# clearmatics/libff

Hardware: AMD Instinct MI355X
Metric: G1 MSM throughput (scalar-muls/sec) (higher is better)
Workload: dtype u32

## Files before the change

libff_amd/csrc/engine.cpp:

```cpp
#include "../../include/amdmsm.h"
#include "engine_internal.h"
#include "group_vtable.h"
#include "fr_vtable.h"

#include <hip/hip_runtime.h>

#include <fcntl.h>
#include <sys/stat.h>
#include <unistd.h>

#include <algorithm>
#include <atomic>
#include <cmath>
#include <cstdio>
#include <cstdlib>
#include <cstring>
#include <initializer_list>
#include <mutex>
#include <string>
#include <thread>
#include <utility>
#include <vector>

using namespace amdmsm;

constexpr int MAX_SLOTS = 4;
constexpr int MAX_GROUPS = 4;
struct ws_slot {
    void *ws = nullptr;
    size_t ws_bytes = 0;
    hipEvent_t done = nullptr;
    bool used = false;
    hipStream_t side[MAX_GROUPS - 1] = {};
    hipEvent_t acc_done[MAX_GROUPS - 1] = {}, tail_done[MAX_GROUPS - 1] = {};
    long long last_ticket = -1;
    bool ev_valid = false;
    hipEvent_t ov_in = nullptr, ov_acc = nullptr, ov_tail = nullptr;
};

struct grow_buf {
    void *p = nullptr;
    size_t bytes = 0;
};

struct base_entry {
    uint64_t id = 0;
    int curve = 0, group = 0, form = 0;
    const char *host = nullptr;
    size_t n = 0, stride = 0;
    void *d_aff = nullptr;
    void *d_endo = nullptr;
    bool automatic = false;
    bool pinned = false;
    uint64_t last_use = 0;
    size_t aff_bytes = 0;
    size_t bytes() const { return n * aff_bytes * (d_endo ? 2 : 1); }
};

struct fb_state {
    grow_buf small, table, table_aff, out;
    bool valid = false;
    int curve = 0, group = 0;
    size_t scalar_size = 0, window = 0;
    unsigned char g[3 * 24 * 2 * 4] = {};
};

struct stream_state {
    static constexpr int NB = 2;
    void *h_stage[NB] = {};
    size_t h_bytes[NB] = {};
// ... 284 lines not shown
    place(p.big, &off, batch, p.c <= 22 ? align_up(std::max(sort_geometry(n, p.c, p.W).big_words, big_words_min) * 4, 256) : 256);
    place(p.tmp_payload, &off, Wt, p.list_stride * 4);
    place(p.tmp_key, &off, Wt, p.list_stride * 4);
    place(p.endo, &off, batch, glv ? align_up((n / 2) * (size_t)vt->el_words * 2 * 4, 256) : 0);
    {
        static const int rc_env = getenv("AMDMSM_ROWCOL") ? atoi(getenv("AMDMSM_ROWCOL")) : 1;
        static const int rc_min_c = getenv("AMDMSM_ROWCOL_MIN_C") ? atoi(getenv("AMDMSM_ROWCOL_MIN_C")) : 10;
        static const int qr_env = getenv("AMDMSM_ROWCOL_QROW") ? atoi(getenv("AMDMSM_ROWCOL_QROW")) : 0;
        static const int qc_env = getenv("AMDMSM_ROWCOL_QCOL") ? atoi(getenv("AMDMSM_ROWCOL_QCOL")) : 0;
        p.rowcol = rc_env != 0 && p.c >= rc_min_c;
        const int h = p.c / 2;
        const size_t C = (size_t)1 << h, R = p.B >> h;
        const bool one_wave = vt->fq_words >= 24 || vt->el_words > vt->fq_words;
        const size_t lane_budget = one_wave ? 70000 : 140000;
        uint32_t q = 4;
        while (q < 64 && Wt * p.B * red_lanes * 2 / q > lane_budget) q <<= 1;
        p.q_row = qr_env > 0 ? (uint32_t)qr_env : q;
        p.q_col = qc_env > 0 ? (uint32_t)qc_env : q;
        place(p.rc, &off, Wt, (R + 1 + C) * xyz_bytes);
        place(p.planes, &off, Wt, p.c * xyz_bytes);
        place(p.winsum, &off, Wt, xyz_bytes);
    }
    p.total = off;
    return AMDMSM_OK;
}

int ensure_ws(amdmsm_ctx *ctx, ws_slot &sl, size_t bytes) {
    if (sl.ws_bytes >= bytes) return AMDMSM_OK;
    if (sl.ws) {
        HIP_TRY(ctx, hipDeviceSynchronize());
        HIP_TRY(ctx, hipFree(sl.ws));
        sl.ws = nullptr;
        sl.ws_bytes = 0;
    }
    const size_t want = bytes + bytes / 8;
    HIP_TRY(ctx, hipMalloc(&sl.ws, want));
    sl.ws_bytes = want;
    return AMDMSM_OK;
}

constexpr uint64_t TIMING_RING = 64;
hipError_t timing_event(hipEvent_t *e) {
    static const bool nofence = !(getenv("AMDMSM_TIMING_NOFENCE") && atoi(getenv("AMDMSM_TIMING_NOFENCE")) == 0);
    return nofence ? hipEventCreateWithFlags(e, hipEventDisableSystemFence) : hipEventCreate(e);
}
void record(amdmsm_ctx *ctx, ws_slot &, int idx, hipStream_t st) {
    if (ctx->timing) (void)hipEventRecord(ctx->ring[ctx->ticket % TIMING_RING][idx], st);
}

int glv_env() {
    static const int env = [] {
        const char *e = getenv("AMDMSM_GLV");
        int v = 0;
        if (!e) return 0;
        if (!strcmp(e, "off") || !strcmp(e, "0")) v = -1;
        else if (!strcmp(e, "on") || !strcmp(e, "1")) v = 1;
        else if (!strcmp(e, "all") || !strcmp(e, "force") || !strcmp(e, "2")) v = 2;
        else if (!strcmp(e, "auto")) v = 3;
        if (v) fprintf(stderr, "[amdmsm] AMDMSM_GLV=%s overrides amdmsm_opts.endomorphism where the caller left it at 0 "
                               "(off: everywhere); on / force assert that every base lies in the order-r subgroup\n", e);
        return v;
    }();
    return env;
}
int endomorphism_permitted(const group_vtable *vt, const amdmsm_opts *opts) {
    const int env = glv_env();
// ... 38 lines not shown
    return (opts && opts->stream) ? (hipStream_t)opts->stream : ctx->stream;
}
amdmsm_opts opts_or_default(const amdmsm_opts *opts) {
    amdmsm_opts o = AMDMSM_OPTS_INIT;
    if (opts) o = *opts;
    else o.out_form = AMDMSM_OUT_LIBFF;
    return o;
}

constexpr size_t MAX_RANGES = 64;
size_t max_range_points() {
    static const size_t v = [] {
        const char *e = getenv("AMDMSM_MAX_RANGE_POINTS");
        const long long x = e ? atoll(e) : 0;
        return x > 0 ? (size_t)x : (size_t)1 << 28;
    }();
    return v;
}

struct msm_hook {
    int (*fn)(void *arg, hipEvent_t *wait_for) = nullptr;
    void *arg = nullptr;
};
struct short_spec {
    int kind = 0;
    int bits = 0;
    uint32_t *flag = nullptr;
    bool uploaded = false;
    size_t elem_bytes(const group_vtable *vt) const { return kind ? (size_t)kind : (size_t)vt->fr_words * 4; }
};
int short_limit_bits(const group_vtable *vt, const short_spec &ss) {
    return ss.flag ? ss.bits : (ss.kind ? 8 * ss.kind : 32 * vt->fr_words);
}
uint32_t *enqueue_tail(const group_vtable *vt, const plan_t &p, char *ws, int w0, int nw, hipStream_t ts, int queue) {
    const size_t w = (size_t)w0;
    uint32_t *buckets = ws_at(ws, p.buckets, w);
    vt->accumulate_fixup(ts, ws_at(ws, p.counts, w), buckets, ws_at(ws, p.pfirst, w), ws_at(ws, p.plast, w), ws_at(ws, p.cont, w),
                         ws_at(ws, p.queue, (size_t)queue), nw, p.B, p.S, p.T);
    if (p.rowcol) {
        uint32_t *winsum = ws_at(ws, p.winsum, w);
        vt->reduce_rowcol(ts, buckets, nw, p.B, p.c, p.q_row, p.q_col, ws_at(ws, p.rc, w), ws_at(ws, p.planes, w), winsum);
        return winsum;
    }
    uint32_t *src = ws_at(ws, p.lvl0, w), *dst = ws_at(ws, p.lvl1, w);
    vt->reduce_segments(ts, buckets, nw, p.B, p.L, src);
    const uint32_t fold = (uint32_t)vt->reduce_fold;
    uint32_t M = p.B / p.L;
    M /= std::min<uint32_t>(M, fold);
    while (M > 1) {
        if ((size_t)M * (64 / fold) <= 256) {
            vt->sum_block(ts, src, nw, M, dst);
            M = 1;
        } else {
            vt->sum_butterfly(ts, src, nw, M, dst);
            M /= std::min<uint32_t>(M, fold);
        }
        std::swap(src, dst);
    }
    return src;
}

int msm_device_impl(amdmsm_ctx *ctx, const group_vtable *vt, const uint32_t *d_bases, const uint32_t *d_scalars,
                    size_t n, uint32_t *d_out, const amdmsm_opts *opts, int table_digits = 0,
                    const msm_hook *hook = nullptr, const uint32_t *d_endo_resident = nullptr, const short_spec *ss = nullptr) {
    hipStream_t st = stream_of(ctx, opts);
    hipStream_t const user_st = st;
    const int form = opts ? opts->out_form : AMDMSM_OUT_LIBFF;
    const int mont = (opts && opts->scalars_plain) ? 0 : 1;
    static const bool atomic_env = getenv("AMDMSM_SORT") && !strcmp(getenv("AMDMSM_SORT"), "atomic");
    const bool atomic_sort = atomic_env && !ss;
    const bool glv = !ss && use_endomorphism(vt, n, opts, table_digits) && !atomic_sort;
// ... 5 lines not shown
        return AMDMSM_OK;
    }
    plan_t p;
    static const int acc_s_env = getenv("AMDMSM_ACC_S") ? atoi(getenv("AMDMSM_ACC_S")) : 0;
    static const int groups_env = getenv("AMDMSM_WINDOW_GROUPS") ? atoi(getenv("AMDMSM_WINDOW_GROUPS")) : 0;
    static const bool overlap_env = getenv("AMDMSM_OVERLAP") && atoi(getenv("AMDMSM_OVERLAP")) != 0;
    const bool overlap = overlap_env && ctx->depth > 1 && ctx->bulk_stream && vt->accumulate_overlap_ok && !groups_env;
    plan_req req;
    req.entries = entries;
    req.c = opts ? opts->window_bits : 0;
    req.L = opts ? opts->segment_len : 0;
    req.S = acc_s_env;
    req.table_digits = table_digits;
    req.groups = groups_env;
    req.glv = glv;
    req.overlap = overlap;
    req.sbits = ss ? ss->bits : 0;
    int rc = make_plan(vt, req, p);
    if (rc) return fail(ctx, rc, "bad window_bits / segment_len");
    if (ss && p.c > 22) return fail(ctx, AMDMSM_ERR_BAD_ARG, "window_bits > 22 is not available for short scalars");
    const int slot_idx = (int)(ctx->next++ % (unsigned)ctx->depth);
    ws_slot &sl = ctx->slots[slot_idx];
    ctx->last_slot = slot_idx;
    if (overlap) {
        HIP_TRY(ctx, hipEventRecord(sl.ov_in, user_st));
        st = ctx->bulk_stream;
        HIP_TRY(ctx, hipStreamWaitEvent(st, sl.ov_in, 0));
    }
    if (sl.used) HIP_TRY(ctx, hipStreamWaitEvent(st, sl.done, 0));
    rc = ensure_ws(ctx, sl, p.total);
    if (rc) return rc;
    char *ws = (char *)sl.ws;
    const sort_bufs sb = sort_bufs_of(p, ws, 0);

    record(ctx, sl, 0, st);
    const uint32_t *endo_pts = !glv ? nullptr : (d_endo_resident ? d_endo_resident : ws_at(ws, p.endo));
    const bool endo_beside = glv && !d_endo_resident && !(hook && hook->fn);
    HIP_TRY(ctx, hipEventRecord(sl.tail_done[0], st));
    if ((atomic_sort || p.c > 22) && !table_digits) {
        HIP_TRY(ctx, hipMemsetAsync(sb.ends, 0, (size_t)p.W * p.counts.unit, st));
        vt->count(st, d_scalars, n, mont, p.c, p.W, sb.ends);
        record(ctx, sl, 1, st);
        vt->scatter(st, d_scalars, n, mont, p.c, p.W, sb.ends, sb.lists, p.list_stride);
    } else {
        HIP_TRY(ctx, hipMemsetAsync(sb.coarse, 0, p.big.off + 16 - p.coarse.off, st));
        record(ctx, sl, 1, st);
        if (ss)
            vt->sort(st, sort_src::short_scalars(d_scalars, ss->kind, short_limit_bits(vt, *ss), ss->flag), n, mont, p.c, p.W, sb, 0);
        else
            vt->sort(st, sort_src::own(d_scalars), n, mont, p.c, table_digits ? table_digits : p.W, sb,
                     table_digits ? 1 : (glv ? 2 : 0));
    }
    hipStream_t side = overlap ? st : sl.side[0];
    if (!overlap) HIP_TRY(ctx, hipStreamWaitEvent(side, sl.tail_done[0], 0));
    HIP_TRY(ctx, hipMemsetAsync(ws_at(ws, p.buckets), 0, (size_t)p.W * p.buckets.unit, side));
    for (int g = 0; g < p.G; ++g) HIP_TRY(ctx, hipMemsetAsync(ws_at(ws, p.queue, (size_t)g), 0, 8, side));
    if (endo_beside) vt->endo_points(side, d_bases, n, ws_at(ws, p.endo));
    if (!overlap) HIP_TRY(ctx, hipEventRecord(sl.acc_done[0], side));
    if (hook && hook->fn) {
        hipEvent_t wait_for = nullptr;
        rc = hook->fn(hook->arg, &wait_for);
        if (rc) return rc;
        if (wait_for) HIP_TRY(ctx, hipStreamWaitEvent(st, wait_for, 0));
    }
    if (!overlap) HIP_TRY(ctx, hipStreamWaitEvent(st, sl.acc_done[0], 0));
    if (glv && !d_endo_resident && !endo_beside) vt->endo_points(st, d_bases, n, ws_at(ws, p.endo));
    int w_hi = p.W;
    for (int g = 0; g < p.G; ++g) {
        const int wg = p.W / p.G + (g < p.W % p.G ? 1 : 0);
        const int w0 = w_hi - wg;
        w_hi = w0;
        const bool last = g == p.G - 1;
        hipStream_t ts = last ? (overlap ? ctx->tail_stream : st) : sl.side[g];
        if (g == 0) record(ctx, sl, 2, st);
        vt->accumulate(st, ws_at(ws, p.counts, w0), ws_at(ws, p.lists, w0), p.list_stride, d_bases, ws_at(ws, p.buckets, w0),
                       ws_at(ws, p.pfirst, w0), ws_at(ws, p.plast, w0), ws_at(ws, p.cont, w0), wg, p.B, p.S, p.T, endo_pts, n,
                       overlap ? 1 : 0);
        if (last) {
            record(ctx, sl, 3, st);
            if (overlap) {
                HIP_TRY(ctx, hipEventRecord(sl.ov_acc, st));
                HIP_TRY(ctx, hipStreamWaitEvent(ts, sl.ov_acc, 0));
            }
        } else {
            HIP_TRY(ctx, hipEventRecord(sl.acc_done[g], st));
            HIP_TRY(ctx, hipStreamWaitEvent(ts, sl.acc_done[g], 0));
        }
        const uint32_t *src = enqueue_tail(vt, p, ws, w0, wg, ts, g);
        if (g > 0) HIP_TRY(ctx, hipStreamWaitEvent(ts, sl.tail_done[g - 1], 0));
        if (last) record(ctx, sl, 4, ts);
        vt->horner(ts, src, wg, p.c, last ? form : (int)AMDMSM_OUT_JACOBIAN, g > 0 ? ws_at(ws, p.partial, g - 1) : nullptr,
                   last ? d_out : ws_at(ws, p.partial, g));
        if (!last) HIP_TRY(ctx, hipEventRecord(sl.tail_done[g], ts));
    }
    if (overlap) {
        record(ctx, sl, 5, ctx->tail_stream);
        HIP_TRY(ctx, hipEventRecord(sl.ov_tail, ctx->tail_stream));
        HIP_TRY(ctx, hipStreamWaitEvent(user_st, sl.ov_tail, 0));
        st = user_st;
    } else {
        record(ctx, sl, 5, st);
    }
    if (ctx->timing) sl.last_ticket = (long long)ctx->ticket++;
    sl.ev_valid = ctx->timing;
    HIP_TRY(ctx, hipEventRecord(sl.done, st));
    sl.used = true;
    HIP_TRY(ctx, hipGetLastError());
    return AMDMSM_OK;
}

constexpr int MAX_BATCH = 8;
int ensure_buf(amdmsm_ctx *ctx, grow_buf &b, size_t bytes);

struct item_dev {
    const uint32_t *bases = nullptr;
    size_t n = 0;
    const uint32_t *scalars = nullptr;
    size_t offset = 0;
    const uint32_t *index = nullptr;
    uint32_t *out = nullptr;
};

int msm_device_batch_items_impl(amdmsm_ctx *ctx, const group_vtable *vt, int k, const item_dev *it, const uint32_t *d_shared,
                                size_t shared_n, uint32_t *flags, const amdmsm_opts *opts) {
    hipStream_t st = stream_of(ctx, opts);
    const int form = opts ? opts->out_form : AMDMSM_OUT_LIBFF;
    const int mont = (opts && opts->scalars_plain) ? 0 : 1;
    size_t n_max = 0;
    for (int j = 0; j < k; ++j) n_max = std::max(n_max, it[j].n);
    if (flags) HIP_TRY(ctx, hipMemsetAsync(flags, 0, (size_t)k * 4, st));
    if (n_max == 0) {
        for (int j = 0; j < k; ++j) vt->sum_points(st, it[j].out, 0, form, it[j].out);
        HIP_TRY(ctx, hipGetLastError());
        return AMDMSM_OK;
    }
    const bool glv = use_endomorphism(vt, n_max, opts, 0);
    const size_t entries = glv ? 2 * n_max : n_max;
    plan_req req;
    req.entries = entries;
    req.c = opts ? opts->window_bits : 0;
    req.L = opts ? opts->segment_len : 0;
    req.glv = glv;
    req.batch = k;
    plan_t p;
    int rc = make_plan(vt, req, p);
    if (rc) return fail(ctx, rc, "bad window_bits / segment_len");
    if (p.c > 22) return fail(ctx, AMDMSM_ERR_BAD_ARG, "window_bits > 22 is not available for a batch");
    req.c = p.c;
    for (int j = 0; j < k; ++j) {
        if (it[j].n) req.big_words_min = std::max(req.big_words_min, sort_geometry(glv ? 2 * it[j].n : it[j].n, p.c, p.W).big_words);
    }
    rc = make_plan(vt, req, p);
    if (rc) return fail(ctx, rc, "bad window_bits / segment_len");
    const int slot_idx = (int)(ctx->next++ % (unsigned)ctx->depth);
    ws_slot &sl = ctx->slots[slot_idx];
    ctx->last_slot = slot_idx;
    if (sl.used) HIP_TRY(ctx, hipStreamWaitEvent(st, sl.done, 0));
    rc = ensure_ws(ctx, sl, p.total);
    if (rc) return rc;
    char *ws = (char *)sl.ws;
    const size_t Wt = (size_t)p.W * (size_t)k;
    record(ctx, sl, 0, st);
    HIP_TRY(ctx, hipMemsetAsync(ws_at(ws, p.coarse), 0, p.big.off - p.coarse.off, st));
    for (int j = 0; j < k; ++j) HIP_TRY(ctx, hipMemsetAsync(ws_at(ws, p.big, (size_t)j), 0, 16, st));
    HIP_TRY(ctx, hipMemsetAsync(ws_at(ws, p.buckets), 0, Wt * p.buckets.unit, st));
    HIP_TRY(ctx, hipMemsetAsync(ws_at(ws, p.queue), 0, 8, st));
    record(ctx, sl, 1, st);
    bool first = true;
    for (int j = 0; j < k; ++j) {
        const size_t w0 = (size_t)j * p.W, n = it[j].n;
        const sort_bufs sb = sort_bufs_of(p, ws, (size_t)j);
        if (n == 0) {
            HIP_TRY(ctx, hipMemsetAsync(sb.ends, 0, (size_t)p.W * p.counts.unit, st));
            HIP_TRY(ctx, hipMemsetAsync(ws_at(ws, p.cont, w0), 0xff, (size_t)p.W * p.cont.unit, st));
            continue;
        }
        const sort_src src_j = it[j].scalars ? sort_src::own(it[j].scalars)
                                             : sort_src::selected(d_shared, shared_n, it[j].index, it[j].offset, flags + j);
        vt->sort(st, src_j, n, mont, p.c, p.W, sb, glv ? 2 : 0);
        uint32_t *endo_j = glv ? ws_at(ws, p.endo, (size_t)j) : nullptr;
        if (glv) vt->endo_points(st, it[j].bases, n, endo_j);
        if (first) record(ctx, sl, 2, st);
        first = false;
        vt->accumulate(st, sb.ends, sb.lists, p.list_stride, it[j].bases, ws_at(ws, p.buckets, w0), ws_at(ws, p.pfirst, w0),
                       ws_at(ws, p.plast, w0), ws_at(ws, p.cont, w0), p.W, p.B, p.S, p.T, endo_j, n, 0);
    }
    record(ctx, sl, 3, st);
    const uint32_t *src = enqueue_tail(vt, p, ws, 0, (int)Wt, st, 0);
    record(ctx, sl, 4, st);
    uint32_t *outs[MAX_BATCH];
// ... 1929 lines not shown

struct vec_opts {
    int mont, form, kernel_form;
};
vec_opts vec_opts_of(const amdmsm_opts *opts) {
    const int form = opts ? opts->out_form : AMDMSM_OUT_LIBFF;
    return {(opts && opts->scalars_plain) ? 0 : 1, form, form == AMDMSM_OUT_AFFINE ? (int)AMDMSM_OUT_LIBFF : form};
}
void vec_finish(const group_vtable *vt, hipStream_t st, const vec_opts &vo, uint32_t *d_xyz, size_t n, uint32_t *scratch) {
    if (vo.form != AMDMSM_OUT_AFFINE) return;
    vt->import_bases(st, d_xyz, (size_t)vt->el_words * 3, 0, n, scratch);
    vt->export_affine(st, scratch, n, d_xyz);
}

int vec_check_stride(amdmsm_ctx *ctx, const group_vtable *vt, size_t &stride_bytes, const char *what) {
    const size_t xyz_bytes = (size_t)vt->el_words * 12;
    if (stride_bytes == 0) stride_bytes = xyz_bytes;
    if (stride_bytes % rec_align(vt) || stride_bytes < xyz_bytes) return fail(ctx, AMDMSM_ERR_BAD_ARG, what);
    return AMDMSM_OK;
}
int vec_upload(amdmsm_ctx *ctx, const group_vtable *vt, hipStream_t st, const void *points_xyz, size_t stride_bytes, int base_form,
               size_t first, size_t m, void *d_aff) {
    HIP_TRY(ctx, hipMemcpyAsync(ctx->hb_src.p, (const char *)points_xyz + first * stride_bytes,
                                (m - 1) * stride_bytes + (size_t)vt->el_words * 12, hipMemcpyHostToDevice, st));
    vt->import_bases(st, (const uint32_t *)ctx->hb_src.p, stride_bytes / 4, base_form == AMDMSM_FORM_SPECIAL, m, (uint32_t *)d_aff);
    return AMDMSM_OK;
}

int slot_begin(amdmsm_ctx *ctx, hipStream_t st, size_t bytes, ws_slot *&slp) {
    const int slot_idx = (int)(ctx->next++ % (unsigned)ctx->depth);
    ws_slot &sl = ctx->slots[slot_idx];
    ctx->last_slot = slot_idx;
    if (sl.used) HIP_TRY(ctx, hipStreamWaitEvent(st, sl.done, 0));
    slp = &sl;
    return ensure_ws(ctx, sl, bytes);
}
int slot_end(amdmsm_ctx *ctx, hipStream_t st, ws_slot &sl) {
    record(ctx, sl, 5, st);
    if (ctx->timing) sl.last_ticket = (long long)ctx->ticket++;
    sl.ev_valid = ctx->timing;
    HIP_TRY(ctx, hipEventRecord(sl.done, st));
    sl.used = true;
    return AMDMSM_OK;
}

template <class Chunk>
int vec_run_chunks(amdmsm_ctx *ctx, const group_vtable *vt, hipStream_t st, size_t ws_bytes, size_t n, size_t cn, void *h_out,
                   Chunk &&chunk) {
    const size_t xyz_bytes = (size_t)vt->el_words * 12;
    ws_slot *sl = nullptr;
    int rc = slot_begin(ctx, st, ws_bytes, sl);
    if (rc) return rc;
    record(ctx, *sl, 0, st);
    for (size_t off = 0; off < n; off += cn) {
        const size_t m = n - off < cn ? n - off : cn;
        rc = chunk(*sl, off, m, off == 0);
        if (rc) {
            if (h_out) (void)hipDeviceSynchronize();
            return rc;
        }
        if (h_out) HIP_TRY(ctx, hipMemcpyAsync((char *)h_out + off * xyz_bytes, ctx->fb.out.p, m * xyz_bytes, hipMemcpyDeviceToHost, st));
        if (off == 0) record(ctx, *sl, 4, st);
        if (h_out) HIP_TRY(ctx, hipStreamSynchronize(st));
    }
    return slot_end(ctx, st, *sl);
}
// ... 1941 lines not shown
```

libff_amd/csrc/group_vtable.h:

```cpp
#pragma once
#include <hip/hip_runtime_api.h>
#include <stddef.h>
#include <stdint.h>
#include <stdlib.h>

namespace amdmsm {

enum out_form : int {
    OUT_JACOBIAN = 0,
    OUT_LIBFF = 1,
    OUT_AFFINE = 2,
};

struct sort_geom {
    int hb;
    int fb;
    uint32_t chunk_cap;
    uint32_t big_thresh;
    uint32_t big_cap;
    size_t big_words;
};
constexpr int SORT_HB_MAX = 10;
constexpr size_t SORT_COARSE_WORDS = ((size_t)1 << SORT_HB_MAX) + 1, SORT_CURSOR_WORDS = (size_t)1 << SORT_HB_MAX;
inline sort_geom sort_geometry(size_t n, int c, int W) {
// ... 111 lines not shown
    const uint32_t* glv_lambda;

    void (*import_bases)(hipStream_t, const uint32_t* src, size_t stride_words, int form_special,
                         size_t n, uint32_t* dst_affine);
    void (*export_affine)(hipStream_t, const uint32_t* src_affine, size_t n, uint32_t* dst_xyz);
    void (*gen_bases_seq)(hipStream_t, unsigned long long first, size_t n, uint32_t* dst_affine);
    void (*endo_points)(hipStream_t, const uint32_t* bases_affine, size_t n, uint32_t* out);
    void (*precompute_table)(hipStream_t, const uint32_t* bases_affine, size_t n, int c, int D, uint32_t* tmp,
                             uint32_t* table);
    void (*ffi_decode_points)(hipStream_t, const uint32_t* src_be, size_t n, uint32_t* dst_affine, uint32_t* status);
    void (*ffi_decode_scalars)(hipStream_t, const uint32_t* src_be, size_t n, uint32_t* dst_plain, uint32_t* status);
    void (*ffi_encode_point)(hipStream_t, const uint32_t* src_xyz_affine, uint32_t* dst_be);
    void (*disk_decode)(hipStream_t, const uint32_t* src, size_t n, uint32_t* dst_affine);
    void (*disk_decode_compressed)(hipStream_t, const uint32_t* src, size_t n, uint32_t* dst_affine, uint32_t* status);

    void (*scalar_stats)(hipStream_t, const uint32_t* scalars, size_t n, int mont, uint32_t* stats);
    void (*scalar_bits)(hipStream_t, const void* scalars, int kind, size_t n, int mont, uint32_t* out_bits);
    void (*gather_scalars)(hipStream_t, const uint32_t* shared, size_t shared_n, const uint32_t* index, size_t offset,
                           uint32_t* flag, size_t n, uint32_t* out);
    void (*count)(hipStream_t, const uint32_t* scalars, size_t n, int mont, int c, int W, uint32_t* counts);
    void (*scatter)(hipStream_t, const uint32_t* scalars, size_t n, int mont, int c, int W, uint32_t* cursor,
                    uint32_t* lists, size_t list_stride);
    void (*sort)(hipStream_t, const sort_src& src, size_t n, int mont, int c, int W, const sort_bufs& bufs, int mode);
    int (*sort_top_window)(int mode, int mont, int c, int W, size_t columns, int* tb);

    void (*accumulate)(hipStream_t, const uint32_t* ends, const uint32_t* lists, size_t list_stride,
                       const uint32_t* bases_affine, uint32_t* buckets, uint32_t* part_first, uint32_t* part_last,
                       uint32_t* cont_bucket, int W, uint32_t B, uint32_t S, uint32_t T, const uint32_t* endo_points,
                       size_t n_real, int overlap);
    size_t (*accumulate_resident_lanes)(int overlap);
    int accumulate_overlap_ok;
    void (*accumulate_fixup)(hipStream_t, const uint32_t* ends, uint32_t* buckets, uint32_t* part_first,
                             const uint32_t* part_last, const uint32_t* cont_bucket, uint32_t* queue, int W,
                             uint32_t B, uint32_t S, uint32_t T);

    void (*reduce_segments)(hipStream_t, const uint32_t* buckets, int W, uint32_t B, uint32_t L, uint32_t* out);
    void (*sum_butterfly)(hipStream_t, const uint32_t* in, int W, uint32_t M, uint32_t* out);
    void (*sum_block)(hipStream_t, const uint32_t* in, int W, uint32_t M, uint32_t* out);
    void (*reduce_rowcol)(hipStream_t, const uint32_t* buckets, int W, uint32_t B, int c, uint32_t q_row, uint32_t q_col,
                          uint32_t* rc, uint32_t* planes, uint32_t* out);
    void (*horner)(hipStream_t, const uint32_t* window_sums, int W, int c, int form, const uint32_t* init,
                   uint32_t* out);
    void (*horner_batch)(hipStream_t, const uint32_t* window_sums, int k, int W, int c, int form, uint32_t* const* outs);
    void (*sum_points)(hipStream_t, const uint32_t* pts, int k, int form, uint32_t* out);

    void (*fixed_base_exp)(hipStream_t, const uint32_t* g_xyz, int scalar_size, int window, const uint32_t* scalars,
                           size_t n, int mont, const uint32_t* coeff, int form, uint32_t* gouter, uint32_t* table,
                           uint32_t* table_aff, int build_table, uint32_t* out);

    int smv_entries;
    void (*smv_table)(hipStream_t, const uint32_t* bases_affine, size_t n, uint32_t* tmp, uint32_t* table);
    void (*smv_ladder)(hipStream_t, const uint32_t* table, size_t n, const uint32_t* scalars, int mont, int form, uint32_t* out);

    int seg_windows, seg_digit_stride;
    void (*seg_digits)(hipStream_t, const uint32_t* scalars, size_t n, int mont, uint32_t* digits);
    void (*seg_accumulate)(hipStream_t, const uint32_t* table, size_t nt, const uint32_t* digits, const uint32_t* slices,
                           size_t n_slices, uint32_t* sums);
    void (*seg_fold)(hipStream_t, const uint32_t* sums, const uint32_t* seg_first, size_t m, uint32_t* winsum);
    void (*seg_horner)(hipStream_t, const uint32_t* winsum, size_t m, int form, uint32_t* out);

    int fold_digit_stride;
    void (*fold_digits)(hipStream_t, const uint32_t* scalars_host, int k, int mont, int glv, int W, uint32_t* digits);
    void (*fold_ladder)(hipStream_t, const uint32_t* tables, size_t n, const uint32_t* digits, int rows, int glv, int W,
                        int form, uint32_t* out);

    void (*fft_gather)(hipStream_t, const uint32_t* in_affine, size_t b0, size_t cn, int rsh, uint32_t* dst_affine);
    void (*fft_butterfly)(hipStream_t, const uint32_t* table, size_t cn, const uint32_t* in_affine, size_t b0, int rsh,
// ... 43 lines not shown
```

libff_amd/csrc/msm_group.hip:

```cpp
#include "curve_params.h"
#include "ec.cuh"
#include "fp2h.cuh"
#include "group_vtable.h"
#include "wide.cuh"
#include "wide28.cuh"
#include "rr.cuh"

#include <algorithm>
#include <cstdio>
#include <vector>
#include <type_traits>

#ifndef AMDMSM_GROUP
#error "compile with -DAMDMSM_GROUP=<group traits> -DAMDMSM_VT=<vtable getter name>"
#endif

namespace amdmsm {
template <bool I>
struct ec_coeff_a<Fp<AMDMSM_GROUP::fq, I>> {
    static constexpr int value = AMDMSM_GROUP::DEG == 1 ? AMDMSM_GROUP::COEFF_A : 0;
};
template <int NR, bool I>
struct ec_coeff_a<Fp2<AMDMSM_GROUP::fq, NR, I>> {
    static constexpr int value = AMDMSM_GROUP::DEG == 2 ? AMDMSM_GROUP::COEFF_A : 0;
// ... 868 lines not shown
    __shared__ uint32_t tmp[NT / 64 + 1];
    const uint32_t nbin = 1u << hb;
    const uint32_t bin = blockIdx.x, w = blockIdx.y;
    const bool top = dtop != 0 && w == gridDim.y - 1u;
    const int fb = c - 1 - hb - (top ? dtop : 0);
    const uint32_t nfine = 1u << fb, fmask = nfine - 1u;
    uint32_t* fstart = smem;
    uint32_t* chist = fstart + nfine;
    uint32_t* cstart = chist + nfine;
    uint32_t* ccur = cstart + nfine;
    uint32_t* st_payload = ccur + nfine;
    unsigned short* st_fine = reinterpret_cast<unsigned short*>(st_payload + chunk_cap);
    const uint32_t* cs = coarse + (size_t)w * (nbin + 1);
    const uint32_t b0 = __builtin_amdgcn_readfirstlane(cs[bin]), m = __builtin_amdgcn_readfirstlane(cs[bin + 1]) - b0;
    const sort_key_t* key = tmp_key + (size_t)w * stride + b0;
    const uint32_t* pay = tmp_payload + (size_t)w * stride + b0;
    uint32_t* out = lists + (size_t)w * stride + b0;
    uint32_t* e = ends + (((size_t)w << (c - 1)) + ((size_t)bin << fb));
    if (top) {
        const uint32_t share = (1u << (fb + dtop)) - nfine, total = cs[nbin];
        uint32_t* tail = ends + (((size_t)w << (c - 1)) + ((size_t)nbin << fb) + (size_t)bin * share);
        for (uint32_t j = threadIdx.x; j < share; j += NT) tail[j] = total;
    }
    if (m > big_thresh) {
        for (uint32_t j = threadIdx.x; j < nfine; j += NT) e[j] = 0;
        if (threadIdx.x == 0) {
            const uint32_t tiles = (m + SORT_TILE - 1) / SORT_TILE;
            const uint32_t slot = atomicAdd(&big[0], 1u);
            uint32_t* rec = big + 4 + 4 * (size_t)slot;
            rec[0] = w;
            rec[1] = bin;
            rec[2] = atomicAdd(&big[1], tiles);
            rec[3] = tiles;
        }
        return;
    }
    if (m <= chunk_cap) {
        uint32_t fr[PER];
        if (m == 0) {
            for (uint32_t j = threadIdx.x; j < nfine; j += NT) e[j] = b0;
            return;
        }
        for (uint32_t j = threadIdx.x; j < nfine; j += NT) chist[j] = 0;
#pragma unroll
        for (int q = 0; q < PER; ++q) {
            const uint32_t k = threadIdx.x + (uint32_t)q * NT;
            fr[q] = (uint32_t)key[k < m ? k : m - 1u] & fmask;
        }
        __syncthreads();
#pragma unroll
        for (int q = 0; q < PER; ++q) {
            const uint32_t k = threadIdx.x + (uint32_t)q * NT;
            const uint32_t r = k < m ? atomicAdd(&chist[fr[q]], 1u) : 0u;
            fr[q] = r | (fr[q] << 14);
        }
        __syncthreads();
        block_exclusive_scan<NT, (1 << SORT_MAX_FB) / NT>(chist, fstart, nfine, tmp);
        for (uint32_t j = threadIdx.x; j < nfine; j += NT) e[j] = b0 + fstart[j] + chist[j];
#pragma unroll
        for (int q = 0; q < PER; ++q) {
            const uint32_t k = threadIdx.x + (uint32_t)q * NT;
            if (k < m) st_payload[fstart[fr[q] >> 14] + (fr[q] & 0x3fffu)] = pay[k];
        }
        __syncthreads();
        for (uint32_t k = threadIdx.x; k < m; k += NT) out[k] = st_payload[k];
        return;
// ... 49 lines not shown
        }
        __syncthreads();
        for (uint32_t j = threadIdx.x; j < nfine; j += NT) fstart[j] += hist_c[j];
        __syncthreads();
    }
}

struct big_tile {
    uint32_t rec, w, bin, k0, cm;
};
AMDMSM_DEV bool big_find_tile(const uint32_t* __restrict__ big, const uint32_t* __restrict__ coarse, uint32_t nbin,
                              uint32_t tile, uint32_t* sh, big_tile& bt, uint32_t& b0) {
    const uint32_t nbig = big[0];
    __syncthreads();
    for (uint32_t r = threadIdx.x; r < nbig; r += SORT_TPB) {
        const uint32_t* rec = big + 4 + 4 * (size_t)r;
        if (tile >= rec[2] && tile < rec[2] + rec[3]) sh[0] = r;
    }
    __syncthreads();
    bt.rec = sh[0];
    const uint32_t* rec = big + 4 + 4 * (size_t)bt.rec;
    bt.w = rec[0];
    bt.bin = rec[1];
    const uint32_t* cs = coarse + (size_t)bt.w * (nbin + 1);
    b0 = cs[bt.bin];
    const uint32_t m = cs[bt.bin + 1] - b0;
    bt.k0 = (tile - rec[2]) * SORT_TILE;
    bt.cm = (m - bt.k0 < (uint32_t)SORT_TILE) ? m - bt.k0 : (uint32_t)SORT_TILE;
    return true;
}

__global__ void __launch_bounds__(SORT_TPB) k_sort_big_hist(const sort_key_t* __restrict__ tmp_key,
                                                            const uint32_t* __restrict__ coarse, size_t stride, int c,
                                                            int hb, const uint32_t* __restrict__ big,
                                                            uint32_t* __restrict__ ends, uint32_t wtop, int dtop) {
    __shared__ uint32_t hist[1 << SORT_MAX_FB], sh[1];
    const uint32_t nbin = 1u << hb;
    const uint32_t tiles = big[1];
    for (uint32_t tile = blockIdx.x; tile < tiles; tile += gridDim.x) {
        big_tile bt;
        uint32_t b0;
        big_find_tile(big, coarse, nbin, tile, sh, bt, b0);
        const int fb = c - 1 - hb - (bt.w == wtop ? dtop : 0);
        const uint32_t nfine = 1u << fb, fmask = nfine - 1u;
        for (uint32_t j = threadIdx.x; j < nfine; j += SORT_TPB) hist[j] = 0;
        __syncthreads();
        const sort_key_t* key = tmp_key + (size_t)bt.w * stride + b0 + bt.k0;
        for (uint32_t k = threadIdx.x; k < bt.cm; k += SORT_TPB) atomicAdd(&hist[key[k] & fmask], 1u);
        __syncthreads();
        uint32_t* e = ends + (((size_t)bt.w << (c - 1)) + ((size_t)bt.bin << fb));
        for (uint32_t j = threadIdx.x; j < nfine; j += SORT_TPB)
            if (hist[j]) atomicAdd(&e[j], hist[j]);
    }
}

__global__ void __launch_bounds__(SORT_TPB) k_sort_big_scan(const uint32_t* __restrict__ coarse, int c, int hb,
                                                            uint32_t big_cap, uint32_t* __restrict__ big,
                                                            uint32_t* __restrict__ ends, uint32_t wtop, int dtop) {
    __shared__ uint32_t cnt[1 << SORT_MAX_FB], out[1 << SORT_MAX_FB], tmp[SORT_TPB / 64 + 1];
    const uint32_t nbin = 1u << hb;
    const int fb_row = c - 1 - hb;
    const uint32_t nbig = big[0];
    for (uint32_t r = blockIdx.x; r < nbig; r += gridDim.x) {
        const uint32_t* rec = big + 4 + 4 * (size_t)r;
        const uint32_t w = rec[0], bin = rec[1];
        const uint32_t b0 = coarse[(size_t)w * (nbin + 1) + bin];
        const int fb = fb_row - (w == wtop ? dtop : 0);
        const uint32_t nfine = 1u << fb;
        uint32_t* e = ends + (((size_t)w << (c - 1)) + ((size_t)bin << fb));
        uint32_t* cur = big + 4 + 4 * (size_t)big_cap + ((size_t)r << fb_row);
        __syncthreads();
        for (uint32_t j = threadIdx.x; j < nfine; j += SORT_TPB) cnt[j] = e[j];
        __syncthreads();
        block_exclusive_scan(cnt, out, nfine, tmp);
        for (uint32_t j = threadIdx.x; j < nfine; j += SORT_TPB) {
            cur[j] = b0 + out[j];
            e[j] = b0 + out[j] + cnt[j];
        }
    }
}

__global__ void __launch_bounds__(SORT_TPB, SORT_WAVES_2WG) k_sort_big_scatter(const uint32_t* __restrict__ tmp_payload,
                                                               const sort_key_t* __restrict__ tmp_key,
                                                               const uint32_t* __restrict__ coarse, size_t stride, int c,
                                                               int hb, uint32_t big_cap, uint32_t* __restrict__ big,
// ... 420 lines not shown
        acc_add(acc, pi >= n_real ? endo_pts + (size_t)(pi - n_real) * AFFW : bases + (size_t)pi * AFFW, (ent >> 31) != 0);
    }
#endif
    if (bend == hi) {
        acc_store(from_prev ? part_first + g * ZZS : bk + (size_t)b * ZZS, acc);
        cont_bucket[g] = NO_BUCKET;
    } else if (from_prev) {
        acc_store(part_first + g * ZZS, acc);
        cont_bucket[g] = NO_BUCKET;
    } else {
        acc_store(part_last + g * ZZS, acc);
        cont_bucket[g] = b;
    }
}

AMDMSM_DEV void wave_group_sum(Jac<E>& p, uint32_t G);
AMDMSM_DEV void wave_group_sum_r(Jac<ER>& p, uint32_t G);

#ifdef AMDMSM_INLINE_SPAN
constexpr uint32_t INLINE_SPAN = AMDMSM_INLINE_SPAN;
#else
constexpr uint32_t INLINE_SPAN = FQ::N <= 8 ? 3 : 2;
#endif
constexpr uint32_t MID_SPAN = 32;
constexpr uint32_t MID_G = 8;

AMDMSM_DEV uint32_t* fixup_queue_base(uint32_t* q, size_t lanes, int mid) {
    return q + 2 + (mid ? 2 * fixup_queue_cap_long(lanes) : 0);
}

AMDMSM_DEV void fixup_compact_block(uint32_t blk, const uint32_t* __restrict__ ends, uint32_t* __restrict__ part_first, int W,
                                    uint32_t B, uint32_t S, uint32_t T);

__global__ void __launch_bounds__(64, AMDMSM_TAIL_WAVES) k_accumulate_fixup(const uint32_t* __restrict__ ends,
                                                         uint32_t* __restrict__ part_first,
                                                         const uint32_t* __restrict__ part_last,
                                                         const uint32_t* __restrict__ cont_bucket,
                                                         uint32_t* __restrict__ buckets, uint32_t* __restrict__ queue,
                                                         int W, uint32_t B, uint32_t S, uint32_t T, uint32_t fix_blocks) {
    if (blockIdx.x >= fix_blocks) {
        fixup_compact_block(blockIdx.x - fix_blocks, ends, part_first, W, B, S, T);
        return;
    }
    const size_t g = gtid() / RED_LANES;
    const bool first_of_pair = (threadIdx.x % RED_LANES) == 0;
    const size_t w = g / T;
    const uint32_t t = (uint32_t)(g % T);
    uint32_t b = NO_BUCKET, t_last = 0;
    if (w < (size_t)W) {
        b = cont_bucket[g];
        if (b != NO_BUCKET) t_last = (ends[w * B + b] - 1) / S;
    }
    const uint32_t span = (b != NO_BUCKET) ? t_last - t : 0;
    const size_t lanes = (size_t)W * T;
#pragma unroll
    for (int mid = 0; mid < 2; ++mid) {
        const bool mine = first_of_pair && (mid ? (span > INLINE_SPAN && span <= MID_SPAN) : (span > MID_SPAN));
        const unsigned long long m = __ballot(mine);
        if (m == 0) continue;
        const uint32_t lane = threadIdx.x & 63u;
        uint32_t base = 0;
        if (lane == (uint32_t)__ffsll((long long)m) - 1u) base = atomicAdd(&queue[mid], (uint32_t)__popcll(m));
        base = (uint32_t)__shfl((int)base, __ffsll((long long)m) - 1, 64);
        if (mine) {
            const uint32_t slot = base + (uint32_t)__popcll(m & ((1ull << lane) - 1ull));
            uint32_t* q = fixup_queue_base(queue, lanes, mid);
            q[2 * (size_t)slot] = (uint32_t)g;
            q[2 * (size_t)slot + 1] = (uint32_t)(g >> 32);
        }
    }
    if (span == 0 || span > INLINE_SPAN) return;
    rec_sum sum;
// ... 1872 lines not shown
    if (split_hist && sg.chunk_cap >= 16384 && ((size_t)16 << sg.fb) * 4 <= 32768) perchunk_words = 16u << sg.fb;
    const size_t fine_lds = ((size_t)4 << sg.fb) * 4 + (size_t)sg.chunk_cap * 6 + (size_t)perchunk_words * 4;
    const size_t big_lds = ((size_t)4 << sg.fb) * 4 + (size_t)SORT_TILE * 4;
    static const bool reported = [&] {
        if (!(getenv("AMDMSM_SORT_REPORT") && atoi(getenv("AMDMSM_SORT_REPORT")))) return false;
        int k16 = 0, k32 = 0, kf = 0, kb = 0;
        (void)hipOccupancyMaxActiveBlocksPerMultiprocessor(&k16, k_sort_coarse<unsigned short>, SORT_TPB, 0);
        (void)hipOccupancyMaxActiveBlocksPerMultiprocessor(&k32, k_sort_coarse<uint32_t>, SORT_TPB, 0);
        if (sg.chunk_cap <= 8192)
            (void)hipOccupancyMaxActiveBlocksPerMultiprocessor(&kf, k_sort_fine<SORT_TPB, 8>, SORT_TPB, fine_lds);
        else if (sg.chunk_cap <= 12288)
            (void)hipOccupancyMaxActiveBlocksPerMultiprocessor(&kf, k_sort_fine<SORT_TPB, 12>, SORT_TPB, fine_lds);
        else
            (void)hipOccupancyMaxActiveBlocksPerMultiprocessor(&kf, k_sort_fine<SORT_TPB, 16>, SORT_TPB, fine_lds);
        (void)hipOccupancyMaxActiveBlocksPerMultiprocessor(&kb, k_sort_big_scatter, SORT_TPB, big_lds);
        fprintf(stderr, "[amdmsm sort] workgroups per CU: k_sort_coarse 16-bit keys %d, 32-bit keys %d; k_sort_fine<1024> "
                        "(chunk_cap %u, %zu B of LDS) %d; k_sort_big_scatter (%zu B) %d\n",
                k16, k32, sg.chunk_cap, fine_lds, kf, big_lds, kb);
        return true;
    }();
    (void)reported;
#define AMDMSM_LAUNCH_FINE(NT, PER)                                                                                          \
    hipLaunchKernelGGL((k_sort_fine<NT, PER>), dim3(nbin, We), dim3(NT), fine_lds, st, b.tmp_payload, tmp_key16, b.coarse, b.stride, c, \
                       hb, sg.chunk_cap, sg.big_thresh, sg.big_cap, perchunk_words, b.big, b.ends, b.lists, dtop)
    if (sg.chunk_cap <= 4096)
        AMDMSM_LAUNCH_FINE(256, 16);
    else if (sg.chunk_cap <= 8192)
        AMDMSM_LAUNCH_FINE(SORT_TPB, 8);
    else if (sg.chunk_cap <= 12288)
        AMDMSM_LAUNCH_FINE(SORT_TPB, 12);
    else
        AMDMSM_LAUNCH_FINE(SORT_TPB, 16);
#undef AMDMSM_LAUNCH_FINE
    hipLaunchKernelGGL(k_sort_big_hist, dim3(512), dim3(SORT_TPB), 0, st, tmp_key16, b.coarse, b.stride, c, hb, b.big, b.ends, wtop, dtop);
    hipLaunchKernelGGL(k_sort_big_scan, dim3(256), dim3(SORT_TPB), 0, st, b.coarse, c, hb, sg.big_cap, b.big, b.ends, wtop, dtop);
    hipLaunchKernelGGL(k_sort_big_scatter, dim3(512), dim3(SORT_TPB), big_lds, st, b.tmp_payload, tmp_key16, b.coarse, b.stride, c,
                       hb, sg.big_cap, b.big, b.lists, wtop, dtop);
}
void l_scalar_bits(hipStream_t st, const void* scalars, int kind, size_t n, int mont, uint32_t* out) {
    if (!n) return;
    const size_t items = kind == 1 ? packed_items<1>(scalars, n) : kind == 2 ? packed_items<2>(scalars, n)
                         : kind == 4 ? packed_items<4>(scalars, n) : kind == 8 ? packed_items<8>(scalars, n) : n;
    const dim3 grid((unsigned)std::min<size_t>((items + TPB - 1) / TPB, 4096));
    if (kind == 1) hipLaunchKernelGGL(k_scalar_bits<1>, grid, dim3(TPB), 0, st, scalars, n, mont, out);
    else if (kind == 2) hipLaunchKernelGGL(k_scalar_bits<2>, grid, dim3(TPB), 0, st, scalars, n, mont, out);
    else if (kind == 4) hipLaunchKernelGGL(k_scalar_bits<4>, grid, dim3(TPB), 0, st, scalars, n, mont, out);
    else if (kind == 8) hipLaunchKernelGGL(k_scalar_bits<8>, grid, dim3(TPB), 0, st, scalars, n, mont, out);
    else hipLaunchKernelGGL(k_scalar_bits<0>, grid, dim3(TPB), 0, st, scalars, n, mont, out);
}
void l_gather_scalars(hipStream_t st, const uint32_t* shared, size_t shared_n, const uint32_t* index, size_t offset,
                      uint32_t* flag, size_t n, uint32_t* out) {
    if (!n) return;
    hipLaunchKernelGGL(k_gather_scalars, dim3(blocks_for(n)), dim3(TPB), 0, st, shared, n, index, offset, shared_n, flag, out);
}
size_t l_accumulate_resident_lanes(int overlap);
constexpr size_t ACC_OVERLAP_LDS = AMDMSM_ACC_WAVES >= 3 ? (160 * 1024) / AMDMSM_ACC_WAVES - 16 * 1024 + 1024 : 0;
void l_accumulate(hipStream_t st, const uint32_t* ends, const uint32_t* lists, size_t list_stride, const uint32_t* bases,
                  uint32_t* buckets, uint32_t* part_first, uint32_t* part_last, uint32_t* cont_bucket, int W, uint32_t B,
                  uint32_t S, uint32_t T, const uint32_t* endo_pts, size_t n_real, int overlap) {
    overlap = overlap && AMDMSM_OVERLAP_OK && ACC_OVERLAP_LDS;
    int sync_waves = (size_t)W * T * ACC_LANES <= 2 * l_accumulate_resident_lanes(overlap) * ACC_LANES ? 1 : 0;
    if (overlap) sync_waves = 2;
    const size_t dyn_lds = overlap ? ACC_OVERLAP_LDS : 0;
#ifdef AMDMSM_ACC_TRACE
    {
        const size_t waves = (size_t)blocks_for((size_t)W * T * ACC_LANES) * TPB / 64;
        static unsigned long long* d_trace = nullptr;
        static size_t cap = 0;
// ... 13 lines not shown
            if (FILE* f = fopen(path, "wb")) {
                fwrite(h.data(), 8, h.size(), f);
                fclose(f);
            }
        }
    }
#else
    hipLaunchKernelGGL(k_accumulate, dim3(blocks_for((size_t)W * T * ACC_LANES)), dim3(TPB), dyn_lds, st, ends, lists,
                       list_stride, bases, buckets, part_first, part_last, cont_bucket, W, B, S, T, endo_pts,
                       endo_pts ? (uint32_t)n_real : 0x80000000u, sync_waves);
#endif
}
void l_endo_points(hipStream_t st, const uint32_t* bases, size_t n, uint32_t* out) {
    if (!n) return;
    hipLaunchKernelGGL(k_endo_points, dim3(blocks_for(n * 2 * GP::DEG)), dim3(TPB), 0, st, bases, n, out);
}
void l_glv_digits(hipStream_t st, const uint32_t* scalars, size_t n, int mont, int c, int W, int32_t* out) {
    if (!n) return;
    hipLaunchKernelGGL(k_glv_digits, dim3(blocks_for(n)), dim3(TPB), 0, st, scalars, n, mont, c, W, out);
}
size_t l_accumulate_resident_lanes(int overlap) {
    auto query = [](size_t dyn_lds) {
        int dev = 0, cus = 256, blocks = 0;
        if (hipGetDevice(&dev) == hipSuccess) (void)hipDeviceGetAttribute(&cus, hipDeviceAttributeMultiprocessorCount, dev);
        if (hipOccupancyMaxActiveBlocksPerMultiprocessor(&blocks, k_accumulate, TPB, dyn_lds) != hipSuccess || blocks <= 0) blocks = 4;
        return (size_t)cus * (size_t)blocks * TPB / ACC_LANES;
    };
    static const size_t lanes = query(0);
    static const size_t lanes_overlap = (AMDMSM_OVERLAP_OK && ACC_OVERLAP_LDS) ? query(ACC_OVERLAP_LDS) : lanes;
    return overlap ? lanes_overlap : lanes;
}
void l_accumulate_fixup(hipStream_t st, const uint32_t* ends, uint32_t* buckets, uint32_t* part_first,
                        const uint32_t* part_last, const uint32_t* cont_bucket, uint32_t* queue, int W, uint32_t B,
                        uint32_t S, uint32_t T) {
    const unsigned fix_blocks = blocks_for((size_t)W * T * RED_LANES, 64);
    const unsigned compact_blocks = T / FIX_BLOCK >= 2 ? (unsigned)(W * (T / FIX_BLOCK - 1)) : 0u;
    hipLaunchKernelGGL(k_accumulate_fixup, dim3(fix_blocks + compact_blocks), dim3(64), 0, st, ends, part_first,
                       part_last, cont_bucket, buckets, queue, W, B, S, T, fix_blocks);
    const size_t lanes = (size_t)W * T;
    const size_t cap_mid = fixup_queue_cap_mid(lanes) / (RED_FOLD / MID_G) + 1, cap_long = fixup_queue_cap_long(lanes);
    const unsigned mid_blocks = (unsigned)(cap_mid < 8192 ? cap_mid : 8192), long_blocks = (unsigned)(cap_long < 2048 ? cap_long : 2048);
    hipLaunchKernelGGL(k_accumulate_fixup_queue, dim3(mid_blocks + long_blocks), dim3(64), 0, st, ends,
                       part_first, part_last, cont_bucket, buckets, queue, mid_blocks, lanes, B, S, T);
}
void l_reduce_segments(hipStream_t st, const uint32_t* buckets, int W, uint32_t B, uint32_t L, uint32_t* out) {
    hipLaunchKernelGGL(k_reduce_segments, dim3(blocks_for((size_t)W * (B / L) * RED_LANES, 64)), dim3(64), 0, st, buckets, W, B,
                       L, out);
}
void l_sum_butterfly(hipStream_t st, const uint32_t* in, int W, uint32_t M, uint32_t* out) {
    hipLaunchKernelGGL(k_sum_butterfly, dim3(blocks_for((size_t)W * M * RED_LANES, 64)), dim3(64), 0, st, in, W, M, out);
}
void l_sum_block(hipStream_t st, const uint32_t* in, int W, uint32_t M, uint32_t* out) {
    if (M >= 8 && M * RED_LANES <= (uint32_t)SUMW_THREADS && (M & (M - 1)) == 0) {
        hipLaunchKernelGGL(k_sum_block_wide, dim3(W), dim3(SUMW_THREADS), 0, st, in, W, M, out);
        return;
    }
    const unsigned threads = (unsigned)((M * RED_LANES + 63) / 64 * 64);
    hipLaunchKernelGGL(k_sum_block, dim3(W), dim3(threads), 0, st, in, W, M, out);
}
void l_reduce_rowcol(hipStream_t st, const uint32_t* buckets, int W, uint32_t B, int c, uint32_t q_row, uint32_t q_col,
                     uint32_t* rc, uint32_t* planes, uint32_t* out) {
    const int h = c / 2;
    const uint32_t C = 1u << h, R = B >> h;
    auto fit = [](uint32_t len, uint32_t q) {
        if (q < 1) q = 1;
        while (q & (q - 1)) q &= q - 1;
        if (q > len) q = len;
        while (len / q > RED_FOLD) q <<= 1;
        return q;
    };
    q_row = fit(C, q_row);
// ... 224 lines not shown
```

Baseline: 664.7 million.

## Fold sort-buffer clearing into fixup kernel and merge big-bin scan into histogram

Instead of a separate memset of the sort scratch region at the start of each MSM, the fixup kernel of the previous call on the same slot gets extra blocks that zero that region, and the next call skips the memset when the slot is known clean. The big-bin histogram kernel also performs the per-record exclusive scan in whichever block finishes last for that record, using an atomic arrival counter, so the separate k_sort_big_scan launch is dropped. This removes a memset and a kernel launch from the critical path. In exchange it relies on cross-call slot state, threadfence-based last-block detection and extra counter storage in the big buffer, which raises correctness risk.

```diff
diff --git a/libff_amd/csrc/engine.cpp b/libff_amd/csrc/engine.cpp
--- a/libff_amd/csrc/engine.cpp
+++ b/libff_amd/csrc/engine.cpp
@@ -36,6 +36,8 @@
     long long last_ticket = -1;
     bool ev_valid = false;
     hipEvent_t ov_in = nullptr, ov_acc = nullptr, ov_tail = nullptr;
+    const char *clean_at = nullptr;
+    size_t clean_bytes = 0;
 };
 
 struct grow_buf {
@@ -386,6 +388,7 @@
         HIP_TRY(ctx, hipFree(sl.ws));
         sl.ws = nullptr;
         sl.ws_bytes = 0;
+        sl.clean_bytes = 0;
     }
     const size_t want = bytes + bytes / 8;
     HIP_TRY(ctx, hipMalloc(&sl.ws, want));
@@ -490,11 +493,12 @@
 int short_limit_bits(const group_vtable *vt, const short_spec &ss) {
     return ss.flag ? ss.bits : (ss.kind ? 8 * ss.kind : 32 * vt->fr_words);
 }
-uint32_t *enqueue_tail(const group_vtable *vt, const plan_t &p, char *ws, int w0, int nw, hipStream_t ts, int queue) {
+uint32_t *enqueue_tail(const group_vtable *vt, const plan_t &p, char *ws, int w0, int nw, hipStream_t ts, int queue,
+                       void *clear = nullptr, size_t clear_bytes = 0) {
     const size_t w = (size_t)w0;
     uint32_t *buckets = ws_at(ws, p.buckets, w);
     vt->accumulate_fixup(ts, ws_at(ws, p.counts, w), buckets, ws_at(ws, p.pfirst, w), ws_at(ws, p.plast, w), ws_at(ws, p.cont, w),
-                         ws_at(ws, p.queue, (size_t)queue), nw, p.B, p.S, p.T);
+                         ws_at(ws, p.queue, (size_t)queue), nw, p.B, p.S, p.T, (uint32_t *)clear, clear_bytes / 4);
     if (p.rowcol) {
         uint32_t *winsum = ws_at(ws, p.winsum, w);
         vt->reduce_rowcol(ts, buckets, nw, p.B, p.c, p.q_row, p.q_col, ws_at(ws, p.rc, w), ws_at(ws, p.planes, w), winsum);
@@ -566,6 +570,11 @@
     if (rc) return rc;
     char *ws = (char *)sl.ws;
     const sort_bufs sb = sort_bufs_of(p, ws, 0);
+    static const bool chain_clear = !(getenv("AMDMSM_CHAIN_CLEAR") && atoi(getenv("AMDMSM_CHAIN_CLEAR")) == 0);
+    const bool two_level = !((atomic_sort || p.c > 22) && !table_digits);
+    const size_t sort_zero_bytes = p.big.off + 16 - p.coarse.off;
+    const bool sort_is_clean = two_level && chain_clear && sl.clean_bytes == sort_zero_bytes && sl.clean_at == (const char *)sb.coarse;
+    sl.clean_bytes = 0;
 
     record(ctx, sl, 0, st);
     const uint32_t *endo_pts = !glv ? nullptr : (d_endo_resident ? d_endo_resident : ws_at(ws, p.endo));
@@ -577,7 +586,7 @@
         record(ctx, sl, 1, st);
         vt->scatter(st, d_scalars, n, mont, p.c, p.W, sb.ends, sb.lists, p.list_stride);
     } else {
-        HIP_TRY(ctx, hipMemsetAsync(sb.coarse, 0, p.big.off + 16 - p.coarse.off, st));
+        if (!sort_is_clean) HIP_TRY(ctx, hipMemsetAsync(sb.coarse, 0, sort_zero_bytes, st));
         record(ctx, sl, 1, st);
         if (ss)
             vt->sort(st, sort_src::short_scalars(d_scalars, ss->kind, short_limit_bits(vt, *ss), ss->flag), n, mont, p.c, p.W, sb, 0);
@@ -620,7 +629,8 @@
             HIP_TRY(ctx, hipEventRecord(sl.acc_done[g], st));
             HIP_TRY(ctx, hipStreamWaitEvent(ts, sl.acc_done[g], 0));
         }
-        const uint32_t *src = enqueue_tail(vt, p, ws, w0, wg, ts, g);
+        const bool clears = last && two_level && chain_clear;
+        const uint32_t *src = enqueue_tail(vt, p, ws, w0, wg, ts, g, clears ? sb.coarse : nullptr, clears ? sort_zero_bytes : 0);
         if (g > 0) HIP_TRY(ctx, hipStreamWaitEvent(ts, sl.tail_done[g - 1], 0));
         if (last) record(ctx, sl, 4, ts);
         vt->horner(ts, src, wg, p.c, last ? form : (int)AMDMSM_OUT_JACOBIAN, g > 0 ? ws_at(ws, p.partial, g - 1) : nullptr,
@@ -640,6 +650,10 @@
     HIP_TRY(ctx, hipEventRecord(sl.done, st));
     sl.used = true;
     HIP_TRY(ctx, hipGetLastError());
+    if (two_level && chain_clear) {
+        sl.clean_at = (const char *)sb.coarse;
+        sl.clean_bytes = sort_zero_bytes;
+    }
     return AMDMSM_OK;
 }
 
@@ -690,6 +704,7 @@
     ws_slot &sl = ctx->slots[slot_idx];
     ctx->last_slot = slot_idx;
     if (sl.used) HIP_TRY(ctx, hipStreamWaitEvent(st, sl.done, 0));
+    sl.clean_bytes = 0;
     rc = ensure_ws(ctx, sl, p.total);
     if (rc) return rc;
     char *ws = (char *)sl.ws;
@@ -2685,6 +2700,7 @@
     ws_slot &sl = ctx->slots[slot_idx];
     ctx->last_slot = slot_idx;
     if (sl.used) HIP_TRY(ctx, hipStreamWaitEvent(st, sl.done, 0));
+    sl.clean_bytes = 0;
     slp = &sl;
     return ensure_ws(ctx, sl, bytes);
 }
diff --git a/libff_amd/csrc/group_vtable.h b/libff_amd/csrc/group_vtable.h
--- a/libff_amd/csrc/group_vtable.h
+++ b/libff_amd/csrc/group_vtable.h
@@ -167,7 +167,7 @@
     int accumulate_overlap_ok;
     void (*accumulate_fixup)(hipStream_t, const uint32_t* ends, uint32_t* buckets, uint32_t* part_first,
                              const uint32_t* part_last, const uint32_t* cont_bucket, uint32_t* queue, int W,
-                             uint32_t B, uint32_t S, uint32_t T);
+                             uint32_t B, uint32_t S, uint32_t T, uint32_t* clear, size_t clear_words);
 
     void (*reduce_segments)(hipStream_t, const uint32_t* buckets, int W, uint32_t B, uint32_t L, uint32_t* out);
     void (*sum_butterfly)(hipStream_t, const uint32_t* in, int W, uint32_t M, uint32_t* out);
diff --git a/libff_amd/csrc/msm_group.hip b/libff_amd/csrc/msm_group.hip
--- a/libff_amd/csrc/msm_group.hip
+++ b/libff_amd/csrc/msm_group.hip
@@ -924,6 +924,7 @@
             rec[1] = bin;
             rec[2] = atomicAdd(&big[1], tiles);
             rec[3] = tiles;
+            big[4 + 4 * (size_t)big_cap + ((size_t)slot << (c - 1 - hb))] = 0;
         }
         return;
     }
@@ -1039,16 +1040,18 @@
 
 __global__ void __launch_bounds__(SORT_TPB) k_sort_big_hist(const sort_key_t* __restrict__ tmp_key,
                                                             const uint32_t* __restrict__ coarse, size_t stride, int c,
-                                                            int hb, const uint32_t* __restrict__ big,
-                                                            uint32_t* __restrict__ ends, uint32_t wtop, int dtop) {
-    __shared__ uint32_t hist[1 << SORT_MAX_FB], sh[1];
+                                                            int hb, uint32_t* __restrict__ big,
+                                                            uint32_t* __restrict__ ends, uint32_t wtop, int dtop,
+                                                            uint32_t big_cap, int scan) {
+    __shared__ uint32_t hist[1 << SORT_MAX_FB], out[1 << SORT_MAX_FB], tmp[SORT_TPB / 64 + 1], sh[2];
     const uint32_t nbin = 1u << hb;
+    const int fb_row = c - 1 - hb;
     const uint32_t tiles = big[1];
     for (uint32_t tile = blockIdx.x; tile < tiles; tile += gridDim.x) {
         big_tile bt;
         uint32_t b0;
         big_find_tile(big, coarse, nbin, tile, sh, bt, b0);
-        const int fb = c - 1 - hb - (bt.w == wtop ? dtop : 0);
+        const int fb = fb_row - (bt.w == wtop ? dtop : 0);
         const uint32_t nfine = 1u << fb, fmask = nfine - 1u;
         for (uint32_t j = threadIdx.x; j < nfine; j += SORT_TPB) hist[j] = 0;
         __syncthreads();
@@ -1058,6 +1061,22 @@
         uint32_t* e = ends + (((size_t)bt.w << (c - 1)) + ((size_t)bt.bin << fb));
         for (uint32_t j = threadIdx.x; j < nfine; j += SORT_TPB)
             if (hist[j]) atomicAdd(&e[j], hist[j]);
+        if (!scan) continue;
+        uint32_t* cur = big + 4 + 4 * (size_t)big_cap + ((size_t)bt.rec << fb_row);
+        __threadfence();
+        __syncthreads();
+        if (threadIdx.x == 0) sh[1] = atomicAdd(&cur[0], 1u) == big[4 + 4 * (size_t)bt.rec + 3] - 1u;
+        __syncthreads();
+        if (!sh[1]) continue;
+        __threadfence();
+        for (uint32_t j = threadIdx.x; j < nfine; j += SORT_TPB)
+            hist[j] = __hip_atomic_load(&e[j], __ATOMIC_RELAXED, __HIP_MEMORY_SCOPE_AGENT);
+        __syncthreads();
+        block_exclusive_scan(hist, out, nfine, tmp);
+        for (uint32_t j = threadIdx.x; j < nfine; j += SORT_TPB) {
+            cur[j] = b0 + out[j];
+            e[j] = b0 + out[j] + hist[j];
+        }
     }
 }
 
@@ -1544,12 +1563,21 @@
 AMDMSM_DEV void fixup_compact_block(uint32_t blk, const uint32_t* __restrict__ ends, uint32_t* __restrict__ part_first, int W,
                                     uint32_t B, uint32_t S, uint32_t T);
 
+constexpr uint32_t FIX_CLEAR_WORDS = 1024;
 __global__ void __launch_bounds__(64, AMDMSM_TAIL_WAVES) k_accumulate_fixup(const uint32_t* __restrict__ ends,
                                                          uint32_t* __restrict__ part_first,
                                                          const uint32_t* __restrict__ part_last,
                                                          const uint32_t* __restrict__ cont_bucket,
                                                          uint32_t* __restrict__ buckets, uint32_t* __restrict__ queue,
-                                                         int W, uint32_t B, uint32_t S, uint32_t T, uint32_t fix_blocks) {
+                                                         int W, uint32_t B, uint32_t S, uint32_t T, uint32_t fix_blocks,
+                                                         uint32_t compact_blocks, uint32_t* __restrict__ clear,
+                                                         uint32_t clear_words) {
+    if (blockIdx.x >= fix_blocks + compact_blocks) {
+        const uint32_t first = (blockIdx.x - fix_blocks - compact_blocks) * FIX_CLEAR_WORDS;
+        const uint32_t end = clear_words - first < FIX_CLEAR_WORDS ? clear_words : first + FIX_CLEAR_WORDS;
+        for (uint32_t i = first + threadIdx.x; i < end; i += 64) clear[i] = 0;
+        return;
+    }
     if (blockIdx.x >= fix_blocks) {
         fixup_compact_block(blockIdx.x - fix_blocks, ends, part_first, W, B, S, T);
         return;
@@ -3488,8 +3516,11 @@
     else
         AMDMSM_LAUNCH_FINE(SORT_TPB, 16);
 #undef AMDMSM_LAUNCH_FINE
-    hipLaunchKernelGGL(k_sort_big_hist, dim3(512), dim3(SORT_TPB), 0, st, tmp_key16, b.coarse, b.stride, c, hb, b.big, b.ends, wtop, dtop);
-    hipLaunchKernelGGL(k_sort_big_scan, dim3(256), dim3(SORT_TPB), 0, st, b.coarse, c, hb, sg.big_cap, b.big, b.ends, wtop, dtop);
+    static const bool big_merge = !(getenv("AMDMSM_SORT_BIG_MERGE") && atoi(getenv("AMDMSM_SORT_BIG_MERGE")) == 0);
+    hipLaunchKernelGGL(k_sort_big_hist, dim3(512), dim3(SORT_TPB), 0, st, tmp_key16, b.coarse, b.stride, c, hb, b.big, b.ends, wtop, dtop,
+                       sg.big_cap, big_merge ? 1 : 0);
+    if (!big_merge)
+        hipLaunchKernelGGL(k_sort_big_scan, dim3(256), dim3(SORT_TPB), 0, st, b.coarse, c, hb, sg.big_cap, b.big, b.ends, wtop, dtop);
     hipLaunchKernelGGL(k_sort_big_scatter, dim3(512), dim3(SORT_TPB), big_lds, st, b.tmp_payload, tmp_key16, b.coarse, b.stride, c,
                        hb, sg.big_cap, b.big, b.lists, wtop, dtop);
 }
@@ -3569,11 +3600,13 @@
 }
 void l_accumulate_fixup(hipStream_t st, const uint32_t* ends, uint32_t* buckets, uint32_t* part_first,
                         const uint32_t* part_last, const uint32_t* cont_bucket, uint32_t* queue, int W, uint32_t B,
-                        uint32_t S, uint32_t T) {
+                        uint32_t S, uint32_t T, uint32_t* clear, size_t clear_words) {
     const unsigned fix_blocks = blocks_for((size_t)W * T * RED_LANES, 64);
     const unsigned compact_blocks = T / FIX_BLOCK >= 2 ? (unsigned)(W * (T / FIX_BLOCK - 1)) : 0u;
-    hipLaunchKernelGGL(k_accumulate_fixup, dim3(fix_blocks + compact_blocks), dim3(64), 0, st, ends, part_first,
-                       part_last, cont_bucket, buckets, queue, W, B, S, T, fix_blocks);
+    const unsigned clear_blocks = clear ? (unsigned)((clear_words + FIX_CLEAR_WORDS - 1) / FIX_CLEAR_WORDS) : 0u;
+    hipLaunchKernelGGL(k_accumulate_fixup, dim3(fix_blocks + compact_blocks + clear_blocks), dim3(64), 0, st, ends, part_first,
+                       part_last, cont_bucket, buckets, queue, W, B, S, T, fix_blocks, compact_blocks, clear,
+                       (uint32_t)clear_words);
     const size_t lanes = (size_t)W * T;
     const size_t cap_mid = fixup_queue_cap_mid(lanes) / (RED_FOLD / MID_G) + 1, cap_long = fixup_queue_cap_long(lanes);
     const unsigned mid_blocks = (unsigned)(cap_mid < 8192 ? cap_mid : 8192), long_blocks = (unsigned)(cap_long < 2048 ? cap_long : 2048);
```

After: 666.6 million, median of 5. Within noise of the previous version (+0.3%).
